# k-dominik/cluster_tools

Hardware: AMD Instinct MI355X
Metric: Gvoxel/s DT-watershed (node, 1/2/4/8 GPU) + % HBM roofline; VI vs ref (higher is better)
Workload: dtype f32

## Files before the change

### cluster_tools_amd/csrc/ctws_api.cpp

```cpp
#include <hip/hip_runtime.h>

#include <algorithm>
#include <chrono>
#include <type_traits>
#include <cmath>
#include <cstdint>
#include <cstdlib>
#include <cstdio>
#include <climits>
#include <cstring>
#include <memory>
#include <string>
#include <thread>
#include <utility>
#include <vector>

#include "../../include/ctws.h"
#include "ctws_kernels.h"
#include "host_pool.h"

using namespace ctws;

namespace {

// ... 64 lines not shown
        hipEvent_t ev_t0 = nullptr, ev_t1 = nullptr;
        std::vector<hipEvent_t> ev_blk;
    } hslot[2];
    hipStream_t s_in = nullptr, s_out = nullptr;
    DevBuf rl_lab, rl_bits, rl_cnt, rl_offs, rl_out, rl_keys, rl_vals, rl_red;
    DevBuf rl_sorted, rl_uniq, rl_counts, rl_tmp;
    int64_t rl_ntable = 0;
    DevBuf edt_fh;
    DevBuf xface;
    DevBuf ptile;
    DevBuf edt_scratch;
    DevBuf fs_vals, fs_sorted, fs_off, fs_tmp;
    DevBuf sf_ids, sf_bits, sf_desc, sf_stat, sf_seeds, sf_lab, sf_hm, sf_out;
    DevBuf rg_lab, rg_tab, rg_nodes, rg_pairs, rg_w, rg_keys, rg_skeys, rg_sw, rg_sum, rg_out, rg_tmp, rg_red;
    DevBuf ef_lab, ef_data, ef_nodes, ef_edges, ef_out, ef_ekeys, ef_keys, ef_skeys, ef_tmp, ef_red;
    DevBuf ov_lab, ov_rows;
    DevBuf mo_rows, mo_acc;
    DevBuf rf_data, rf_rows, rf_cnt, rf_off, rf_sums, rf_ctab;
    DevBuf ds_in, ds_out, ds_flag;
    std::vector<uint32_t> ds_flags;
    DevBuf rc_lab, rc_objs, rc_list, rc_keys, rc_cent, rc_found, rc_a, rc_b;
    DevBuf if_in, if_out, if_a, if_b, if_taps, if_mm;
    std::vector<double> if_taps_host;
    int64_t sf_n = 0;
    uint64_t sf_lo = 1, sf_hi = 0;
    bool sf_has_bits = false;
    DevBuf tc_P, tc_bits, tc_cnt, tc_offs, tc_woff, tc_red, tc_in, tc_mask, tc_out, tc_raw, tc_tmp, tc_taps;
    DevBuf ev_ka, ev_ca, ev_kb, ev_cb, ev_kp, ev_cp, ev_state, ev_out, ev_stage;
    int64_t ev_cap_a = 0, ev_cap_b = 0, ev_cap_p = 0;
    int stop_after = 0;
    int trace = 0;
    int no_descent = 0;
    int seed_tilecc = 0;
    int no_fallback = 0;
    int force_wide = 0;
    int wide_rerun = 0;
    int sf_sparse = 1;
    int fuse_hist = 1;
    int verify = 1;
    int prep_lds = 0;
    int plateau_fill = 1;
    int output_tile = 1;
    int gauss_w = 0;
    int gauss_yx = 1;
    int words_per_wave = 32;
    int d2h_wgs = 0;
    int pack_threads = 6;
    int unpack_threads = 9;
    std::unique_ptr<ctws_host::WorkerPool> pack_pool, unpack_pool;
    int h2d_mode = 0;
    int h2d_wgs = 64;
    int host_ramp = 1;
    int host_batch_blocks = 0;
    int64_t host_batch_voxels = (int64_t)256 << 20;
    int edt_wz = 0;
    int edt_bits = 1;
    int edt_w = 0;
    int fchunk2[3] = {1, 64, 1};
    int fchunk3[3] = {1, 8, 8};
    int fchunk3_masked[3] = {1, 8, 8};
    int fchunk3_env = 0;
    int fc_cur[3] = {1, 64, 1};
    int cur_max[3] = {0, 0, 0};
    int frontier_grid = 1024;
    int frontier_dir = 1;
    int frontier_reps = 32;
// ... 894 lines not shown
        if (edt_bits && maxX <= 256)
            launch_co(std::integral_constant<int, 4>(), std::true_type());
        else if (edt_bits && maxX <= 512)
            launch_co(std::integral_constant<int, 8>(), std::true_type());
        else if (edt_bits)
            launch_co(std::integral_constant<int, 16>(), std::true_type());
        else if (typed && all_exact && maxX == 256) {
            prep_kernel = 200 + 4;
            k_prep_edt_x_reg<4><<<gx, 256, 0, h->stream>>>(w.desc, w.stat, pp, fin_out, (uint32_t*)w.A);
        } else if (typed && all_exact && maxX == 512) {
            prep_kernel = 200 + 8;
            k_prep_edt_x_reg<8><<<gx, 256, 0, h->stream>>>(w.desc, w.stat, pp, fin_out, (uint32_t*)w.A);
        } else if (typed && all_exact && maxX == 1024) {
            prep_kernel = 200 + 16;
            k_prep_edt_x_reg<16><<<gx, 256, 0, h->stream>>>(w.desc, w.stat, pp, fin_out, (uint32_t*)w.A);
        } else if (typed && maxX <= 256)
            launch_co(std::integral_constant<int, 4>(), std::false_type());
        else if (typed && maxX <= 512)
            launch_co(std::integral_constant<int, 8>(), std::false_type());
        else if (typed && maxX <= 1024)
            launch_co(std::integral_constant<int, 16>(), std::false_type());
        else {
            lds_optin(k_prep_edt_x, 4 * (size_t)maxX * 4);
            k_prep_edt_x<<<gx, 256, 4 * (size_t)maxX * 4, h->stream>>>(w.desc, w.stat, pp, fin_out, (uint32_t*)w.A);
        }
        LAUNCHCHK();
        if (pl.from_seeds) k_fs_active<<<(nb + 255) / 256, 256, 0, h->stream>>>(w.desc, w.stat, nb);
        else k_set_active<<<(nb + 255) / 256, 256, 0, h->stream>>>(w.desc, w.stat, nb);
        LAUNCHCHK();
    }
    mark("prep_edt_x");
    set_timing(h, "prep_kernel", (float)prep_kernel);
    bool packed = true;
    uint32_t max_seeds = 0;
    std::vector<BlockStat> s2(nb);
    const dim3 gsb((unsigned)((maxZ + 255) / 256), nb);
    if (pl.from_seeds) {
        r = pl.sf_fill ? fs_seeds(h, desc, nb, TH, TW, TS, maxH, maxRows, vg, wg, uint64_t())
                       : fs_seeds(h, desc, nb, TH, TW, TS, maxH, maxRows, vg, wg, uint32_t());
        if (r != CTWS_OK) return r;
    } else {
    if (real_edt) {
        EdtRealParams er{{pl.pitchd[0], pl.pitchd[1], pl.pitchd[2]}, pl.dt_2d, real_double ? 1 : 0};
        const int nthr = 64 * 256;
        const int maxL = std::max(maxZ, std::max(maxY, maxX));
        const size_t esz = real_double ? 8 : 4;
        if ((r = grow(h, h->edt_scratch, (size_t)nthr * maxL * (2 * esz + 20))) != CTWS_OK) return r;
        char* scr = (char*)h->edt_scratch.p;
        auto run_real = [&](auto tag) {
            using T = decltype(tag);
            T* tmp = (T*)w.key;
            k_edt_real_init<T><<<vg, 256, 0, h->stream>>>(w.desc, w.stat, er, (const uint32_t*)w.A, tmp);
            for (int a = pl.dt_2d ? 1 : 0; a < 3; ++a)
                k_edt_real_line<T><<<nthr / 256, 256, 0, h->stream>>>(w.desc, w.stat, nb, er, a, tmp, scr, maxL);
            k_edt_real_final<T><<<vg, 256, 0, h->stream>>>(w.desc, w.stat, er, tmp, w.dt, w.smin, w.smax);
        };
        if (real_double) run_real(double());
        else run_real(float());
        LAUNCHCHK();
        if (!pl.dt_2d && pl.nd_ws == 2) {
            dim3 gs((unsigned)maxZ, nb);
            k_dt_slice_stats<<<gs, 256, 0, h->stream>>>(w.desc, w.stat, w.dt, w.smin, w.smax);
            LAUNCHCHK();
        }
    } else {
        auto fit = [](int W, int L) {
// ... 57 lines not shown
        std::fprintf(stderr, "[ctws] edt lower-envelope columns: y %u z %u\n", c[0], c[1]);
    }
    if (pl.pass2 && pl.nd_ws == 2) {
        k_p2_zero_dt<<<vg, 256, 0, h->stream>>>(w.desc, w.stat, w.dt);
        HIPCHK(hipMemsetD32Async((hipDeviceptr_t)w.smin, 0xFFFFFFFFu, (size_t)TS, h->stream));
        HIPCHK(hipMemsetAsync(w.smax, 0, sizeof(uint32_t) * TS, h->stream));
        dim3 gs((unsigned)maxZ, nb);
        k_dt_slice_stats<<<gs, 256, 0, h->stream>>>(w.desc, w.stat, w.dt, w.smin, w.smax);
        LAUNCHCHK();
    }
    mark("edt_yz");

    HmapParams hp{(float)cfg->alpha, (float)(1.0 - cfg->alpha), pl.nd_ws == 2 ? 1 : 0};
    const float* seedmap = w.dt;
    if (pl.seeds_smooth) {
        bool any = false;
        for (int a = (pl.nd_ws == 3 ? 0 : 1); a < 3; ++a) any |= pl.sig_seeds[a] > 0.0;
        if (any) {
            if ((r = run_gauss(h, pl, pl.sig_seeds, false, w.dt, w.sm, nb, maxZ, maxY, maxX, hp, 0)) != CTWS_OK)
                return r;
            seedmap = w.sm;
        }
    }
    mark("smooth_seeds");
    {
        const double sw[3] = {pl.weights_smooth ? pl.sig_weights[0] : 0.0, pl.weights_smooth ? pl.sig_weights[1] : 0.0,
                              pl.weights_smooth ? pl.sig_weights[2] : 0.0};
        if ((r = run_gauss(h, pl, sw, true, w.fin, w.hm, nb, maxZ, maxY, maxX, hp, 1)) != CTWS_OK) return r;
    }
    mark("hmap");

    {
        HIPCHK(hipMemsetAsync(h->ptile.p, 0, sizeof(uint32_t) * (size_t)std::max<int64_t>(TPT, 1), h->stream));
        k_localmax<<<wtg, 256, 0, h->stream>>>(w.desc, w.stat, seedmap, w.cls, w.smax, (uint32_t*)h->ptile.p);
        LAUNCHCHK();
        HIPCHK(hipMemsetAsync(w.fseed, 0, sizeof(uint64_t) * (size_t)TF, h->stream));
        CcArgs ca{seedmap, w.cls, w.P, nullptr, nullptr, 0, w.fseed, nullptr, (const uint32_t*)h->ptile.p};
        if (pl.nd_ws == 3) {
            using T = CcTileM<3, CC_SEED>;
            const dim3 tg(tiles8(cdiv(maxZ, T::TZ) * cdiv(maxY, T::TY) * cdiv(maxX, T::TX)), nb);
            k_tile_cc<3, CC_PLATEAU><<<tg, 256, 0, h->stream>>>(w.desc, w.stat, ca, w.P);
            k_tile_merge<3, CC_PLATEAU><<<dim3(std::min(tg.x, 2048u), tg.y), 256, 0, h->stream>>>(w.desc, w.stat, ca, w.P);
            k_plateau_flag<<<vg, 256, 0, h->stream>>>(w.desc, w.stat, w.cls, w.P);
            if (h->seed_tilecc) {
                k_tile_cc<3, CC_SEED><<<tg, 256, 0, h->stream>>>(w.desc, w.stat, ca, w.PF);
                k_tile_merge<3, CC_SEED><<<dim3(std::min(tg.x, 2048u), tg.y), 256, 0, h->stream>>>(w.desc, w.stat, ca, w.PF);
            } else {
                k_seed_members<3><<<wtg, 256, 0, h->stream>>>(w.desc, w.stat, w.cls, w.P, w.PF, w.fseed, nullptr);
            }
        } else {
            using T = CcTile<2>;
            const dim3 tg(tiles8(cdiv(maxZ, T::TZ) * cdiv(maxY, T::TY) * cdiv(maxX, T::TX)), nb);
            k_tile_cc<2, CC_PLATEAU><<<tg, 256, 0, h->stream>>>(w.desc, w.stat, ca, w.P);
            k_tile_merge<2, CC_PLATEAU><<<dim3(std::min(tg.x, 2048u), tg.y), 256, 0, h->stream>>>(w.desc, w.stat, ca, w.P);
            k_plateau_flag<<<vg, 256, 0, h->stream>>>(w.desc, w.stat, w.cls, w.P);
            if (h->seed_tilecc) {
                k_tile_cc<2, CC_SEED><<<tg, 256, 0, h->stream>>>(w.desc, w.stat, ca, w.PF);
                k_tile_merge<2, CC_SEED><<<dim3(std::min(tg.x, 2048u), tg.y), 256, 0, h->stream>>>(w.desc, w.stat, ca, w.PF);
            } else {
                k_seed_members<2><<<wtg, 256, 0, h->stream>>>(w.desc, w.stat, w.cls, w.P, w.PF, w.fseed,
                                                             (uint32_t*)w.A);
                k_seed_union2<<<dim3(64, nb), 256, 0, h->stream>>>(w.desc, w.stat, w.cls, w.P, (const uint32_t*)w.A,
                                                                   w.PF);
            }
        }
        LAUNCHCHK();
    }
    HIPCHK(hipMemsetAsync(w.W, 0, sizeof(uint64_t) * (size_t)TW, h->stream));
    k_flatten_seeds<<<dim3((unsigned)std::min<int64_t>((TF / nb + 255) / 256 + 1, 4096), nb), 256, 0, h->stream>>>(
        w.desc, w.stat, w.PF, w.fseed, w.W);
    k_bitmap_csum<<<wg, 256, 0, h->stream>>>(w.desc, w.stat, 0, w.W, w.csum);
    k_chunk_scan<<<nb, 256, 0, h->stream>>>(w.desc, w.stat, 0, w.csum, 0);
    k_word_prefix<<<wg, 256, 0, h->stream>>>(w.desc, w.stat, 0, w.W, w.csum, w.Wp);
    k_root_label<<<wg, 256, 0, h->stream>>>(w.desc, w.stat, 0, w.PF, w.W, w.Wp, pl.pass2 ? nullptr : (uint32_t*)w.Bf);
    if (pl.pass2) {
        k_slice_seed_base<<<gsb, 256, 0, h->stream>>>(w.desc, w.stat, w.W, w.Wp, w.soff);
        HIPCHK(hipMemsetAsync(w.hkey, 0xFF, sizeof(uint64_t) * (size_t)TH, h->stream));
        HIPCHK(hipMemsetAsync(w.hpos, 0xFF, sizeof(uint32_t) * (size_t)TH, h->stream));
        k_p2_insert<<<vg, 256, 0, h->stream>>>(w.desc, w.stat, w.hkey, w.hpos, w.PF, w.fseed, w.soff,
                                               (const uint32_t*)h->p2_hint_dev.p);
        HIPCHK(hipMemsetAsync(w.W, 0, sizeof(uint64_t) * (size_t)TW, h->stream));
        const dim3 hg((unsigned)std::min<int64_t>((maxH + 255) / 256, 4096), nb);
        k_p2_roots<<<hg, 256, 0, h->stream>>>(w.desc, w.stat, w.hkey, w.hpos, w.W);
        k_bitmap_csum<<<wg, 256, 0, h->stream>>>(w.desc, w.stat, 0, w.W, w.csum);
        k_chunk_scan<<<nb, 256, 0, h->stream>>>(w.desc, w.stat, 0, w.csum, 0);
        k_word_prefix<<<wg, 256, 0, h->stream>>>(w.desc, w.stat, 0, w.W, w.csum, w.Wp);
        k_root_label<<<wg, 256, 0, h->stream>>>(w.desc, w.stat, 0, nullptr, w.W, w.Wp, (uint32_t*)w.dt);
        LAUNCHCHK();
    }
    }
    {
        HIPCHK(hipMemcpyAsync(s2.data(), w.stat, sizeof(BlockStat) * nb, hipMemcpyDeviceToHost, h->stream));
        HIPCHK(hipStreamSynchronize(h->stream));
        for (auto& s : s2) {
// ... 391 lines not shown
        }
        if (any_plain) k_count_ids<<<dim3(64, nb), 256, 0, h->stream>>>(w.desc, w.stat, w.W);
        LAUNCHCHK();
        mark("output");
    }

    HIPCHK(hipMemcpyAsync(st.data(), w.stat, sizeof(BlockStat) * nb, hipMemcpyDeviceToHost, h->stream));
    std::vector<uint32_t> sbh, inmask, soffh;
    if (pl.pass2) {
        sbh.resize(TS);
        inmask.resize(TS);
        HIPCHK(hipMemcpyAsync(sbh.data(), w.sb, sizeof(uint32_t) * TS, hipMemcpyDeviceToHost, h->stream));
        HIPCHK(hipMemcpyAsync(inmask.data(), w.smin, sizeof(uint32_t) * TS, hipMemcpyDeviceToHost, h->stream));
        if (pl.nd_ws == 2) {
            soffh.resize(TS);
            HIPCHK(hipMemcpyAsync(soffh.data(), w.soff, sizeof(uint32_t) * TS, hipMemcpyDeviceToHost, h->stream));
        }
    }
    HIPCHK(hipStreamSynchronize(h->stream));
    for (size_t i = 1; i < ev; ++i) {
        float ms = 0.f;
        hipEventElapsedTime(&ms, h->events[i - 1], h->events[i]);
        add_timing(h, names[i], ms);
    }
    add_timing(h, "flood_rounds", (float)rounds1);
    add_timing(h, "frontier_iters", (float)fiters);
    add_timing(h, "regrow_iters", (float)fiters2);
    add_timing(h, "flood_fallback", (float)fallback);
    add_timing(h, "regrow_rounds", (float)rounds2);
    add_timing(h, "auto_seeded_blocks", (float)n_auto_blocks);
    add_timing(h, "sf_sparse_blocks", (float)n_sf_sparse);
    add_timing(h, "sf_redo_blocks", (float)n_sf_redo);
    add_timing(h, "hist_fused", counts_ready ? 1.f : 0.f);
    add_timing(h, "flood_kernel_ms", fk1);
    add_timing(h, "flood_packed", packed ? 1.f : 0.f);
    add_timing(h, "flood_tiles_solved", (float)h->flood_tiles);
    add_timing(h, "flood_local_iters", (float)h->flood_iters);
    add_timing(h, "flood_lines_swept", (float)h->flood_lines);
    add_timing(h, "size_filter_kernel_ms", fk2);
    std::vector<int> wide;
    if (packed)
        for (int i = 0; i < nb; ++i)
            if (st[i].active && st[i].dsat) wide.push_back(i);
    auto in_wide = [&](int i) { return std::find(wide.begin(), wide.end(), i) != wide.end(); };
    std::vector<int> redo;
    std::vector<std::vector<uint32_t>> redo_hint;
    if (pl.pass2 && pl.nd_ws == 2) {
        for (int i = 0; i < nb; ++i) {
            if (!st[i].active || in_wide(i)) continue;
            std::vector<uint32_t> so(soffh.begin() + desc[i].sbase, soffh.begin() + desc[i].sbase + desc[i].Z);
            const bool again = desc[i].p2hint < 0 ? (st[i].err & kErrCollision) != 0 : so != h->p2_hints[i];
            if (!again || (st[i].err & ~kErrCollision)) continue;
            if (h->p2_depth > desc[i].Z + 1) continue;
            redo.push_back(i);
            redo_hint.push_back(std::move(so));
        }
    }
    for (int i = 0; i < nb; ++i) {
        blocks[i].status = st[i].active ? CTWS_BLOCK_WRITTEN : (pl.pass2 ? CTWS_BLOCK_EMPTY_PASS2 : CTWS_BLOCK_EMPTY);
        blocks[i].max_label = st[i].active ? st[i].max_label : 0;
        if (pl.from_seeds) {
            uint64_t mx;
            std::memcpy(&mx, &st[i]._p[2], sizeof(mx));
            blocks[i].max_label = mx;
        }
        const uint32_t bare = (st[i].active ? st[i]._p[0] : 1u) && desc[i].id_offset != 0;
// ... 501 lines not shown
            for (int i = 0; i < nb; ++i)
                io[i] = {bb[i].input, bb[i].mask, bb[i].initial_seeds, bb[i].output};
            if ((r = run_batch(h, cfg, pl, bb.data(), io.data(), nb)) != CTWS_OK) return r;
        } else {
            if ((r = run_batch(h, cfg, pl, bb.data(), io.data(), nb)) != CTWS_OK) return r;
        }
        for (int i = 0; i < nb; ++i) {
            blocks[todo[k + i]].status = bb[i].status;
            blocks[todo[k + i]].n_ids = bb[i].n_ids;
            blocks[todo[k + i]].max_label = bb[i].max_label;
        }
        k = e;
    }
    return CTWS_OK;
}

}

extern "C" {

int ctws_abi_version(void) { return CTWS_ABI_VERSION; }

int ctws_open(int device, ctws_handle** out) {
    if (!out) return CTWS_EINVAL;
    *out = nullptr;
    int n = 0;
    if (hipGetDeviceCount(&n) != hipSuccess || n <= 0) return CTWS_EHIP;
    if (device < 0 || device >= n) return CTWS_EINVAL;
    ctws_handle* h = new ctws_handle();
    h->device = device;
    if (const char* t = std::getenv("CTWS_TRACE")) h->trace = std::atoi(t);
    if (const char* t = std::getenv("CTWS_NO_DESCENT")) h->no_descent = std::atoi(t);
    if (const char* t = std::getenv("CTWS_SEED_TILECC")) h->seed_tilecc = std::atoi(t);
    if (const char* t = std::getenv("CTWS_NO_FALLBACK")) h->no_fallback = std::atoi(t);
    if (const char* t = std::getenv("CTWS_FORCE_WIDE")) h->force_wide = std::atoi(t);
    if (const char* t = std::getenv("CTWS_SF_SPARSE")) h->sf_sparse = std::atoi(t);
    if (const char* t = std::getenv("CTWS_FUSE_HIST")) h->fuse_hist = std::atoi(t);
    if (const char* t = std::getenv("CTWS_VERIFY")) h->verify = std::atoi(t);
    if (const char* t = std::getenv("CTWS_PREP_LDS")) h->prep_lds = std::atoi(t);
    if (const char* t = std::getenv("CTWS_EDT_BITS")) h->edt_bits = std::atoi(t);
    if (const char* t = std::getenv("CTWS_FRONTIER_ITERS"))
        h->frontier_max_iters = std::max(0, std::min(kFrontierMaxItersCap, std::atoi(t)));
    if (const char* t = std::getenv("CTWS_GAUSS_YX")) h->gauss_yx = std::atoi(t);
    if (const char* t = std::getenv("CTWS_HOST_BATCH_VOXELS")) h->host_batch_voxels = std::max<int64_t>(1, std::atoll(t));
    if (const char* t = std::getenv("CTWS_HOST_RAMP")) h->host_ramp = std::atoi(t);
    if (const char* t = std::getenv("CTWS_PLATEAU_FILL")) h->plateau_fill = std::atoi(t);
    if (const char* t = std::getenv("CTWS_OUTPUT_TILE")) h->output_tile = std::atoi(t);
    if (const char* t = std::getenv("CTWS_H2D_MODE")) h->h2d_mode = std::atoi(t);
    if (const char* t = std::getenv("CTWS_H2D_WGS")) h->h2d_wgs = std::max(1, std::atoi(t));
    if (const char* t = std::getenv("CTWS_HOST_BATCH_BLOCKS")) h->host_batch_blocks = std::max(0, std::atoi(t));
    if (const char* t = std::getenv("CTWS_PACK_THREADS")) h->pack_threads = std::max(1, std::atoi(t));
    if (const char* t = std::getenv("CTWS_UNPACK_THREADS")) h->unpack_threads = std::max(1, std::atoi(t));
    if (const char* t = std::getenv("CTWS_D2H_WGS")) h->d2h_wgs = std::max(0, std::atoi(t));
    if (const char* t = std::getenv("CTWS_WORDS_PER_WAVE")) h->words_per_wave = std::max(1, std::atoi(t));
    if (const char* t = std::getenv("CTWS_GAUSS_W")) {
        const int v = std::atoi(t);
        h->gauss_w = (v == 8 || v == 16 || v == 32) ? v : 0;
    }
    if (const char* t = std::getenv("CTWS_EDT_W")) {
        const int v = std::atoi(t);
        h->edt_w = (v == 8 || v == 16 || v == 32 || v == 64) ? v : 0;
    }
    if (const char* t = std::getenv("CTWS_EDT_WZ")) {
        const int v = std::atoi(t);
        h->edt_wz = (v == 8 || v == 16 || v == 32 || v == 64) ? v : 0;
    }
// ... 2222 lines not shown
```

### cluster_tools_amd/csrc/ctws_kernels.h

```cpp
#pragma once

#include "ctws_dev.h"

namespace ctws {

struct PrepParams {
    float threshold;
    int invert;
    int agg;
    int px2;
};
struct EdtColParams {
    int axis;
    int p2;
    int final_pass;
    int per_slice;
    uint32_t max_dist;
    int px2;
};
struct EdtRealParams {
    double pitch[3];
    int per_slice;
    int real;
};
// ... 29 lines not shown
__global__ void k_edt_col_bits(const BlockDesc*, BlockStat*, EdtColParams, const EdtRec*, uint32_t*, float*, uint32_t*,
                               uint32_t*, unsigned long long*, uint32_t*);
__global__ void k_edt_col_fh(const BlockDesc*, BlockStat*, EdtColParams, const uint32_t*, const EdtRec*, uint32_t*,
                             float*, uint32_t*, uint32_t*, const unsigned long long*, const uint32_t*);
template <class T>
__global__ void k_edt_real_init(const BlockDesc*, const BlockStat*, EdtRealParams, const uint32_t*, T*);
template <class T>
__global__ void k_edt_real_line(const BlockDesc*, const BlockStat*, int, EdtRealParams, int, T*, char*, int);
template <class T>
__global__ void k_edt_real_final(const BlockDesc*, BlockStat*, EdtRealParams, const T*, float*, uint32_t*, uint32_t*);
__global__ void k_dt_slice_stats(const BlockDesc*, const BlockStat*, const float*, uint32_t*, uint32_t*);
__global__ void k_set_active(const BlockDesc*, BlockStat*, int);

__global__ void k_hmap(const BlockDesc*, const BlockStat*, HmapParams, const float*, const float*, const uint32_t*,
                       const uint32_t*, float*);
template <int W>
__global__ void k_gauss_col(const BlockDesc*, const BlockStat*, GaussParams, HmapParams, const double*, const float*,
                            const float*, const uint32_t*, const uint32_t*, float*);
__global__ void k_gauss_row(const BlockDesc*, const BlockStat*, GaussParams, HmapParams, const double*, const float*,
                            const float*, const uint32_t*, const uint32_t*, float*);
constexpr int kTapSlot = 4096;
constexpr int kGaussMaxR = 12;
template <int W, int R>
__global__ void k_gauss_col_r(const BlockDesc*, const BlockStat*, GaussParams, HmapParams, const double*, const float*,
                              const float*, const uint32_t*, const uint32_t*, float*);
template <int R>
__global__ void k_gauss_row_r(const BlockDesc*, const BlockStat*, GaussParams, HmapParams, const double*, const float*,
                              const float*, const uint32_t*, const uint32_t*, float*);
constexpr int kGaussYxTY = 32;
template <int R>
__global__ void k_gauss_yx(const BlockDesc*, const BlockStat*, int, HmapParams, const double*, const double*,
                           const float*, const float*, const uint32_t*, const uint32_t*, float*);

__global__ void k_localmax(const BlockDesc*, BlockStat*, const float*, uint8_t*, const uint32_t*, uint32_t*);
__global__ void k_plateau_flag(const BlockDesc*, const BlockStat*, uint8_t*, uint32_t*);
__global__ void k_flatten_tile_roots(const BlockDesc*, const BlockStat*, uint32_t*, const uint64_t*, uint64_t*);
__global__ void k_flatten_seeds(const BlockDesc*, const BlockStat*, uint32_t*, const uint64_t*, uint64_t*);
template <int ND>
__global__ void k_seed_members(const BlockDesc*, BlockStat*, const uint8_t*, const uint32_t*, uint32_t*, uint64_t*,
                               uint32_t*);
__global__ void k_seed_union2(const BlockDesc*, const BlockStat*, const uint8_t*, const uint32_t*, const uint32_t*,
                              uint32_t*);

__global__ void k_plat_mark(const BlockDesc*, const BlockStat*, const float*, const uint32_t*, uint64_t*, uint64_t*);
template <int ND>
__global__ void k_plat_entry(const BlockDesc*, const BlockStat*, const float*, uint64_t*, const uint64_t*,
                             const uint32_t*);
__global__ void k_plat_scan_x(const BlockDesc*, const BlockStat*, uint64_t*, const uint64_t*, const uint32_t*);
template <int AX>
__global__ void k_plat_scan_col(const BlockDesc*, const BlockStat*, uint64_t*, const uint64_t*, const uint32_t*);
__global__ void k_plat_restore(const BlockDesc*, const BlockStat*, uint64_t*, const uint64_t*, uint64_t*);
__global__ void k_bitmap_csum(const BlockDesc*, const BlockStat*, int, const uint64_t*, uint32_t*);
__global__ void k_chunk_scan(const BlockDesc*, BlockStat*, int, uint32_t*, int);
__global__ void k_word_prefix(const BlockDesc*, const BlockStat*, int, const uint64_t*, const uint32_t*, uint32_t*);
__global__ void k_root_label(const BlockDesc*, const BlockStat*, int, uint32_t*, const uint64_t*, const uint32_t*,
                             uint32_t*);
__global__ void k_seed_label(const BlockDesc*, const BlockStat*, const uint32_t*, const uint64_t*, const float*,
                             uint32_t*, uint64_t*, uint8_t*, int);
__global__ void k_output(const BlockDesc*, BlockStat*, const uint32_t*, const uint64_t*, int, const uint32_t*,
                         const uint32_t*, const uint32_t*, unsigned long long*, int);
__global__ void k_count_ids(const BlockDesc*, BlockStat*, const uint64_t*);

enum CcMode { CC_PLATEAU = 0, CC_SEED = 1, CC_CROP = 2 };
struct CcArgs {
    const float* v;
    const uint8_t* cls;
    const uint32_t* Pp;
    const uint32_t* lab;
// ... 335 lines not shown
```

### cluster_tools_amd/csrc/k_cc.hip

```cpp
#include "ctws_kernels.h"

namespace ctws {

#define BLOCK_LOOP(i, B)                                                                      \
    for (int64_t i = (int64_t)blockIdx.x * blockDim.x + threadIdx.x; i < (B).N;              \
         i += (int64_t)gridDim.x * blockDim.x)

#define ROW_TILES(nz, ny, nx, ...)                                                           \
    {                                                                                         \
        const int64_t nrows_ = (int64_t)(nz) * (ny);                                          \
        for (int64_t r0_ = (int64_t)blockIdx.x * kRows; r0_ < nrows_; r0_ += (int64_t)gridDim.x * kRows) \
            for (int x = threadIdx.x; x < (nx); x += blockDim.x) {                           \
                _Pragma("unroll") for (int rr_ = 0; rr_ < kRows; ++rr_) {                      \
                    const int64_t row_ = r0_ + rr_;                                           \
                    if (row_ >= nrows_) break;                                                \
                    const int z = (int)(row_ / (ny));                                         \
                    const int y = (int)(row_ - (int64_t)z * (ny));                            \
                    const int64_t i = row_ * (nx) + x;                                        \
                    (void)z;                                                                  \
                    (void)y;                                                                  \
                    __VA_ARGS__                                                               \
                }                                                                             \
            }                                                                                 \
    }

template <int ND>
__device__ __forceinline__ void localmax_words(const BlockDesc& B, const BlockStat& st, const uint32_t* __restrict__ smax,
                                               const float* __restrict__ p, uint8_t* __restrict__ cl, uint32_t& nplat,
                                               uint32_t* __restrict__ ptile) {
    const uint32_t ord0 = 0x80000000u;
    constexpr int U = 8, R = U + 2;
    const int Y = B.Y, X = B.X, Z = B.Z;
    const int64_t YX = (int64_t)Y * X;
    const int wpr = (X + 63) >> 6;
    const int ngy = (Y + U - 1) / U;
    const int64_t nunits = (int64_t)Z * wpr * ngy;
    const int lane = threadIdx.x & 63;
    const int64_t nwaves = (int64_t)gridDim.x * (blockDim.x >> 6);
    const int64_t per = (nunits + nwaves - 1) / nwaves;
    const int64_t wid = (int64_t)xcd_swizzle((int)blockIdx.x, (int)gridDim.x) * (blockDim.x >> 6) + (threadIdx.x >> 6);
    const int64_t ubeg = wid * per, uend = min(nunits, ubeg + per);
    const float NEG = -__builtin_huge_valf();
    const gptr_t<float> gp = gbl(p);
    for (int64_t un = ubeg; un < uend; ++un) {
        const uint32_t un32 = (uint32_t)un;
        const int gy = (int)(un32 % (uint32_t)ngy);
        const uint32_t strip = un32 / (uint32_t)ngy;
        const int xw = (int)(strip % (uint32_t)wpr), z = (int)(strip / (uint32_t)wpr);
        const int y0 = gy * U;
        bool ueq = false;
        const int x = xw * 64 + lane;
        const int xc = min(x, X - 1);
        const int xe = lane == 0 ? max(xc - 1, 0) : min(xc + 1, X - 1);
        const int64_t zb = (int64_t)z * YX;
        float rc[R], re[R];
#pragma unroll
        for (int k = 0; k < R; ++k) {
            const int yy = min(max(y0 - 1 + k, 0), Y - 1);
            rc[k] = gp[zb + (int64_t)yy * X + xc];
            re[k] = gp[zb + (int64_t)yy * X + xe];
        }
        float zm[U], zp[U];
// ... 34 lines not shown
            float w[8];
            if (ND == 3) {
                w[0] = z > 0 ? zm[u] : NEG;
                w[1] = z + 1 < Z ? zp[u] : NEG;
                w[2] = yl ? rc[k - 1] : NEG;
                w[3] = yh ? rc[k + 1] : NEG;
                w[4] = xl ? lft[k] : NEG;
                w[5] = xh ? rgt[k] : NEG;
                w[6] = w[7] = NEG;
            } else {
                w[0] = yl && xl ? lft[k - 1] : NEG;
                w[1] = yl ? rc[k - 1] : NEG;
                w[2] = yl && xh ? rgt[k - 1] : NEG;
                w[3] = xl ? lft[k] : NEG;
                w[4] = xh ? rgt[k] : NEG;
                w[5] = yh && xl ? lft[k + 1] : NEG;
                w[6] = yh ? rc[k + 1] : NEG;
                w[7] = yh && xh ? rgt[k + 1] : NEG;
            }
            bool gt = false, eq = false;
#pragma unroll
            for (int q = 0; q < 8; ++q) {
                gt |= w[q] > cc;
                eq |= w[q] == cc;
            }
            if (cc == 0.0f && pos) {
                gt = true;
                eq = false;
            }
            const bool valid = y < Y && x < X;
            if (valid) cl[zb + (int64_t)y * X + x] = (uint8_t)((gt ? 1 : 0) | (eq ? 2 : 0));
            nplat += valid && eq;
            ueq |= valid && eq;
        }
        const uint64_t em = __ballot(ueq);
        if (em && lane < (ND == 3 ? 2 : 1)) {
            using PT = CcTileM<ND, CC_PLATEAU>;
            const int ntx = (X + PT::TX - 1) / PT::TX, nty = (Y + PT::TY - 1) / PT::TY;
            const uint64_t half = ND == 3 ? ((em >> (32 * lane)) & 0xFFFFFFFFull) : em;
            const int txi = ND == 3 ? 2 * xw + lane : xw;
            if (half && txi < ntx) {
                uint32_t* f = ptile + B.ptbase + ((int64_t)(z / PT::TZ) * nty + y0 / PT::TY) * ntx + txi;
                if (!*f) *f = 1u;
            }
        }
    }
}

__global__ void __launch_bounds__(256) k_localmax(const BlockDesc* __restrict__ D, BlockStat* S,
                                                  const float* __restrict__ v, uint8_t* __restrict__ cls,
                                                  const uint32_t* __restrict__ smax, uint32_t* __restrict__ ptile) {
    const BlockDesc& B = D[blockIdx.y];
    if (!S[blockIdx.y].active) return;
    uint32_t nplat = 0;
    if (B.nd_ws == 3) localmax_words<3>(B, S[blockIdx.y], smax, v + B.base, cls + B.base, nplat, ptile);
    else localmax_words<2>(B, S[blockIdx.y], smax, v + B.base, cls + B.base, nplat, ptile);
    nplat = wg_reduce_u32(nplat, OpAdd());
    if (threadIdx.x == 0 && nplat) atomicAdd(&S[blockIdx.y].plateau, nplat);
}

template <int ND>
__global__ void __launch_bounds__(256) k_seed_members(const BlockDesc* __restrict__ D, BlockStat* S,
                                                      const uint8_t* __restrict__ cls, const uint32_t* __restrict__ Pp,
                                                      uint32_t* __restrict__ PFg, uint64_t* __restrict__ fseed,
                                                      uint32_t* __restrict__ plist) {
    const BlockDesc& B = D[blockIdx.y];
    BlockStat& st = S[blockIdx.y];
    if (!st.active) return;
    const bool plat = st.plateau != 0;
    const uint8_t* cl = cls + B.base;
    const uint32_t* PP = Pp + B.base;
    uint32_t* PF = PFg + B.base;
    const int wpr = (B.X + 63) >> 6;
    const int64_t nwords = (int64_t)B.Z * B.Y * wpr;
    const int lane = threadIdx.x & 63;
    const int64_t nwaves = (int64_t)gridDim.x * (blockDim.x >> 6);
    const int64_t per = (nwords + nwaves - 1) / nwaves;
    const int64_t wid = (int64_t)xcd_swizzle((int)blockIdx.x, (int)gridDim.x) * (blockDim.x >> 6) + (threadIdx.x >> 6);
    const int64_t wbeg = wid * per, wend = min(nwords, wbeg + per);
    int row_n = (int)((uint32_t)wbeg / (uint32_t)wpr), xw_n = (int)(wbeg - (int64_t)row_n * wpr);
    constexpr int U = 8;
    for (int64_t w0 = wbeg; w0 < wend; w0 += U) {
        int64_t gi[U];
        bool valid[U];
        uint8_t c[U];
#pragma unroll
        for (int u = 0; u < U; ++u) {
            const int64_t row = row_n;
            const int x = xw_n * 64 + lane;
// ... 76 lines not shown
    const uint32_t n = st._u;
    for (uint32_t e = blockIdx.x * blockDim.x + threadIdx.x; e < n; e += gridDim.x * blockDim.x) {
        const uint32_t i = plist[B.base + e];
        const uint32_t x = i % (uint32_t)B.X, y = (i / (uint32_t)B.X) % (uint32_t)B.Y;
        if (x > 0 && plat_max(i - 1)) unite(i, i - 1);
        if (y > 0 && plat_max(i - (uint32_t)B.X)) unite(i, i - (uint32_t)B.X);
    }
}

__global__ void __launch_bounds__(256) k_plateau_flag(const BlockDesc* __restrict__ D, const BlockStat* S,
                                                      uint8_t* __restrict__ cls, uint32_t* __restrict__ Pg) {
    const BlockDesc& B = D[blockIdx.y];
    if (!S[blockIdx.y].active || !S[blockIdx.y].plateau) return;
    uint8_t* cl = cls + B.base;
    uint32_t* P = Pg + B.base;
    const int64_t a0 = B.base >> 4, a1 = (B.base + B.N + 15) >> 4;
    const uint4* c16 = reinterpret_cast<const uint4*>(cls);
    for (int64_t a = a0 + (int64_t)blockIdx.x * blockDim.x + threadIdx.x; a < a1; a += (int64_t)gridDim.x * blockDim.x) {
        const uint4 q = c16[a];
        const uint32_t wv[4] = {q.x, q.y, q.z, q.w};
#pragma unroll
        for (int k = 0; k < 4; ++k) {
            uint32_t m = wv[k] & (wv[k] >> 1) & 0x01010101u;
            while (m) {
                const int b = __builtin_ctz(m) >> 3;
                m &= m - 1u;
                const int64_t i = a * 16 + k * 4 + b - B.base;
                if (i < 0 || i >= B.N) continue;
                const uint32_t r = uf_find_compress(P, (uint32_t)i);
                cl[r] |= 4;
            }
        }
    }
}

__global__ void __launch_bounds__(256) k_bitmap_csum(const BlockDesc* __restrict__ D, const BlockStat* S, int inner,
                                                     const uint64_t* __restrict__ Wg, uint32_t* __restrict__ csum) {
    const BlockDesc& B = D[blockIdx.y];
    if (!S[blockIdx.y].active || (inner && !B.crop)) return;
    const int64_t n = inner ? B.NI : B.N;
    const int64_t nw = n / 64 + 1;
    if ((int64_t)blockIdx.x * 256 >= nw) return;
    const int64_t w = (int64_t)blockIdx.x * 256 + threadIdx.x;
    uint32_t c = w < nw ? (uint32_t)__popcll(Wg[B.wbase + w]) : 0u;
    for (int s = 32; s > 0; s >>= 1) c += (uint32_t)__shfl_xor((int)c, s);
    __shared__ uint32_t red[4];
    if ((threadIdx.x & 63) == 0) red[threadIdx.x >> 6] = c;
    __syncthreads();
    if (threadIdx.x == 0) csum[B.cbase + blockIdx.x] = red[0] + red[1] + red[2] + red[3];
}

__global__ void __launch_bounds__(256) k_chunk_scan(const BlockDesc* __restrict__ D, BlockStat* S, int inner,
                                                    uint32_t* __restrict__ csum, int which_counter) {
    const BlockDesc& B = D[blockIdx.x];
    if (!S[blockIdx.x].active || (inner && !B.crop)) return;
    const int64_t n = inner ? B.NI : B.N;
    const int64_t nw = n / 64 + 1;
    const int64_t nc = (nw + 255) / 256;
    __shared__ uint32_t tmp[256];
    uint32_t carry = 0;
    for (int64_t c0 = 0; c0 < nc; c0 += 256) {
        const int64_t c = c0 + threadIdx.x;
        uint32_t v = c < nc ? csum[B.cbase + c] : 0u;
        tmp[threadIdx.x] = v;
        __syncthreads();
        for (int s = 1; s < 256; s <<= 1) {
// ... 310 lines not shown
```

Measured before the change: 17.52.

## Emit seed and plateau bitmaps from localmax and process only plateau words

k_localmax now writes per-word ballots of strict local maxima into fseed and of plateau voxels into a new feq bitmap, and writes PF for strict maxima directly. Plateau flagging and seed membership then walk only the nonzero feq words instead of scanning every voxel, and the fseed memset is skipped. The aim is to remove dense full-volume passes over cls in the seed stage. The cost is extra ballot work and global writes inside localmax, plus a new path whose correctness depends on fseed and PF staying consistent. The old dense path stays behind CTWS_SEED_DENSE.

```diff
diff --git a/cluster_tools_amd/csrc/ctws_api.cpp b/cluster_tools_amd/csrc/ctws_api.cpp
--- a/cluster_tools_amd/csrc/ctws_api.cpp
+++ b/cluster_tools_amd/csrc/ctws_api.cpp
@@ -120,6 +120,7 @@
     int trace = 0;
     int no_descent = 0;
     int seed_tilecc = 0;
+    int seed_dense = 0;
     int no_fallback = 0;
     int force_wide = 0;
     int wide_rerun = 0;
@@ -1080,6 +1081,7 @@
     mark("prep_edt_x");
     set_timing(h, "prep_kernel", (float)prep_kernel);
     bool packed = true;
+    const bool seed_dense = !pl.from_seeds && (h->seed_dense || h->seed_tilecc);
     uint32_t max_seeds = 0;
     std::vector<BlockStat> s2(nb);
     const dim3 gsb((unsigned)((maxZ + 255) / 256), nb);
@@ -1203,34 +1205,48 @@
 
     {
         HIPCHK(hipMemsetAsync(h->ptile.p, 0, sizeof(uint32_t) * (size_t)std::max<int64_t>(TPT, 1), h->stream));
-        k_localmax<<<wtg, 256, 0, h->stream>>>(w.desc, w.stat, seedmap, w.cls, w.smax, (uint32_t*)h->ptile.p);
+        const bool dense = seed_dense;
+        uint64_t* const feq = w.fopen;
+        if (dense) k_localmax<<<wtg, 256, 0, h->stream>>>(w.desc, w.stat, seedmap, w.cls, w.smax, (uint32_t*)h->ptile.p,
+                                                         nullptr, nullptr, nullptr);
+        else k_localmax<<<wtg, 256, 0, h->stream>>>(w.desc, w.stat, seedmap, w.cls, w.smax, (uint32_t*)h->ptile.p,
+                                                    w.fseed, feq, w.PF);
         LAUNCHCHK();
-        HIPCHK(hipMemsetAsync(w.fseed, 0, sizeof(uint64_t) * (size_t)TF, h->stream));
+        if (dense) HIPCHK(hipMemsetAsync(w.fseed, 0, sizeof(uint64_t) * (size_t)TF, h->stream));
         CcArgs ca{seedmap, w.cls, w.P, nullptr, nullptr, 0, w.fseed, nullptr, (const uint32_t*)h->ptile.p};
+        const dim3 eg((unsigned)std::min<int64_t>((maxRows * ((maxX + 63) / 64) + 255) / 256, 2048), nb);
         if (pl.nd_ws == 3) {
             using T = CcTileM<3, CC_SEED>;
             const dim3 tg(tiles8(cdiv(maxZ, T::TZ) * cdiv(maxY, T::TY) * cdiv(maxX, T::TX)), nb);
             k_tile_cc<3, CC_PLATEAU><<<tg, 256, 0, h->stream>>>(w.desc, w.stat, ca, w.P);
             k_tile_merge<3, CC_PLATEAU><<<dim3(std::min(tg.x, 2048u), tg.y), 256, 0, h->stream>>>(w.desc, w.stat, ca, w.P);
-            k_plateau_flag<<<vg, 256, 0, h->stream>>>(w.desc, w.stat, w.cls, w.P);
+            if (dense) k_plateau_flag<<<vg, 256, 0, h->stream>>>(w.desc, w.stat, w.cls, w.P);
+            else k_plateau_flag_eq<<<eg, 256, 0, h->stream>>>(w.desc, w.stat, w.cls, w.P, feq);
             if (h->seed_tilecc) {
                 k_tile_cc<3, CC_SEED><<<tg, 256, 0, h->stream>>>(w.desc, w.stat, ca, w.PF);
                 k_tile_merge<3, CC_SEED><<<dim3(std::min(tg.x, 2048u), tg.y), 256, 0, h->stream>>>(w.desc, w.stat, ca, w.PF);
+            } else if (dense) {
+                k_seed_members<3><<<wtg, 256, 0, h->stream>>>(w.desc, w.stat, w.cls, w.P, w.PF, w.fseed, nullptr);
             } else {
-                k_seed_members<3><<<wtg, 256, 0, h->stream>>>(w.desc, w.stat, w.cls, w.P, w.PF, w.fseed, nullptr);
+                k_seed_members_eq<3><<<eg, 256, 0, h->stream>>>(w.desc, w.stat, w.cls, w.P, w.PF, w.fseed, feq, nullptr);
             }
         } else {
             using T = CcTile<2>;
             const dim3 tg(tiles8(cdiv(maxZ, T::TZ) * cdiv(maxY, T::TY) * cdiv(maxX, T::TX)), nb);
             k_tile_cc<2, CC_PLATEAU><<<tg, 256, 0, h->stream>>>(w.desc, w.stat, ca, w.P);
             k_tile_merge<2, CC_PLATEAU><<<dim3(std::min(tg.x, 2048u), tg.y), 256, 0, h->stream>>>(w.desc, w.stat, ca, w.P);
-            k_plateau_flag<<<vg, 256, 0, h->stream>>>(w.desc, w.stat, w.cls, w.P);
+            if (dense) k_plateau_flag<<<vg, 256, 0, h->stream>>>(w.desc, w.stat, w.cls, w.P);
+            else k_plateau_flag_eq<<<eg, 256, 0, h->stream>>>(w.desc, w.stat, w.cls, w.P, feq);
             if (h->seed_tilecc) {
                 k_tile_cc<2, CC_SEED><<<tg, 256, 0, h->stream>>>(w.desc, w.stat, ca, w.PF);
                 k_tile_merge<2, CC_SEED><<<dim3(std::min(tg.x, 2048u), tg.y), 256, 0, h->stream>>>(w.desc, w.stat, ca, w.PF);
             } else {
-                k_seed_members<2><<<wtg, 256, 0, h->stream>>>(w.desc, w.stat, w.cls, w.P, w.PF, w.fseed,
-                                                             (uint32_t*)w.A);
+                if (dense)
+                    k_seed_members<2><<<wtg, 256, 0, h->stream>>>(w.desc, w.stat, w.cls, w.P, w.PF, w.fseed,
+                                                                 (uint32_t*)w.A);
+                else
+                    k_seed_members_eq<2><<<eg, 256, 0, h->stream>>>(w.desc, w.stat, w.cls, w.P, w.PF, w.fseed, feq,
+                                                                   (uint32_t*)w.A);
                 k_seed_union2<<<dim3(64, nb), 256, 0, h->stream>>>(w.desc, w.stat, w.cls, w.P, (const uint32_t*)w.A,
                                                                    w.PF);
             }
@@ -1688,6 +1704,7 @@
     add_timing(h, "sf_sparse_blocks", (float)n_sf_sparse);
     add_timing(h, "sf_redo_blocks", (float)n_sf_redo);
     add_timing(h, "hist_fused", counts_ready ? 1.f : 0.f);
+    add_timing(h, "seed_dense", seed_dense ? 1.f : 0.f);
     add_timing(h, "flood_kernel_ms", fk1);
     add_timing(h, "flood_packed", packed ? 1.f : 0.f);
     add_timing(h, "flood_tiles_solved", (float)h->flood_tiles);
@@ -2255,6 +2272,7 @@
     if (const char* t = std::getenv("CTWS_TRACE")) h->trace = std::atoi(t);
     if (const char* t = std::getenv("CTWS_NO_DESCENT")) h->no_descent = std::atoi(t);
     if (const char* t = std::getenv("CTWS_SEED_TILECC")) h->seed_tilecc = std::atoi(t);
+    if (const char* t = std::getenv("CTWS_SEED_DENSE")) h->seed_dense = std::atoi(t);
     if (const char* t = std::getenv("CTWS_NO_FALLBACK")) h->no_fallback = std::atoi(t);
     if (const char* t = std::getenv("CTWS_FORCE_WIDE")) h->force_wide = std::atoi(t);
     if (const char* t = std::getenv("CTWS_SF_SPARSE")) h->sf_sparse = std::atoi(t);
diff --git a/cluster_tools_amd/csrc/ctws_kernels.h b/cluster_tools_amd/csrc/ctws_kernels.h
--- a/cluster_tools_amd/csrc/ctws_kernels.h
+++ b/cluster_tools_amd/csrc/ctws_kernels.h
@@ -85,8 +85,13 @@
 __global__ void k_gauss_yx(const BlockDesc*, const BlockStat*, int, HmapParams, const double*, const double*,
                            const float*, const float*, const uint32_t*, const uint32_t*, float*);
 
-__global__ void k_localmax(const BlockDesc*, BlockStat*, const float*, uint8_t*, const uint32_t*, uint32_t*);
+__global__ void k_localmax(const BlockDesc*, BlockStat*, const float*, uint8_t*, const uint32_t*, uint32_t*, uint64_t*,
+                           uint64_t*, uint32_t*);
 __global__ void k_plateau_flag(const BlockDesc*, const BlockStat*, uint8_t*, uint32_t*);
+__global__ void k_plateau_flag_eq(const BlockDesc*, const BlockStat*, uint8_t*, uint32_t*, const uint64_t*);
+template <int ND>
+__global__ void k_seed_members_eq(const BlockDesc*, BlockStat*, const uint8_t*, const uint32_t*, uint32_t*, uint64_t*,
+                                  const uint64_t*, uint32_t*);
 __global__ void k_flatten_tile_roots(const BlockDesc*, const BlockStat*, uint32_t*, const uint64_t*, uint64_t*);
 __global__ void k_flatten_seeds(const BlockDesc*, const BlockStat*, uint32_t*, const uint64_t*, uint64_t*);
 template <int ND>
diff --git a/cluster_tools_amd/csrc/k_cc.hip b/cluster_tools_amd/csrc/k_cc.hip
--- a/cluster_tools_amd/csrc/k_cc.hip
+++ b/cluster_tools_amd/csrc/k_cc.hip
@@ -27,7 +27,8 @@
 template <int ND>
 __device__ __forceinline__ void localmax_words(const BlockDesc& B, const BlockStat& st, const uint32_t* __restrict__ smax,
                                                const float* __restrict__ p, uint8_t* __restrict__ cl, uint32_t& nplat,
-                                               uint32_t* __restrict__ ptile) {
+                                               uint32_t* __restrict__ ptile, uint64_t* __restrict__ fseed,
+                                               uint64_t* __restrict__ feq, uint32_t* __restrict__ PF) {
     const uint32_t ord0 = 0x80000000u;
     constexpr int U = 8, R = U + 2;
     const int Y = B.Y, X = B.X, Z = B.Z;
@@ -128,6 +129,16 @@
             if (valid) cl[zb + (int64_t)y * X + x] = (uint8_t)((gt ? 1 : 0) | (eq ? 2 : 0));
             nplat += valid && eq;
             ueq |= valid && eq;
+            if (fseed) {
+                const bool smx = valid && !gt && !eq;
+                const uint64_t ms = __ballot(smx), me = __ballot(valid && eq);
+                if (y < Y && lane == 0) {
+                    const int64_t fw = B.fbase + ((int64_t)z * Y + y) * wpr + xw;
+                    fseed[fw] = ms;
+                    feq[fw] = me;
+                }
+                if (smx) PF[zb + (int64_t)y * X + x] = (uint32_t)(zb + (int64_t)y * X + x);
+            }
         }
         const uint64_t em = __ballot(ueq);
         if (em && lane < (ND == 3 ? 2 : 1)) {
@@ -145,12 +156,15 @@
 
 __global__ void __launch_bounds__(256) k_localmax(const BlockDesc* __restrict__ D, BlockStat* S,
                                                   const float* __restrict__ v, uint8_t* __restrict__ cls,
-                                                  const uint32_t* __restrict__ smax, uint32_t* __restrict__ ptile) {
+                                                  const uint32_t* __restrict__ smax, uint32_t* __restrict__ ptile,
+                                                  uint64_t* __restrict__ fseed, uint64_t* __restrict__ feq,
+                                                  uint32_t* __restrict__ PFg) {
     const BlockDesc& B = D[blockIdx.y];
     if (!S[blockIdx.y].active) return;
     uint32_t nplat = 0;
-    if (B.nd_ws == 3) localmax_words<3>(B, S[blockIdx.y], smax, v + B.base, cls + B.base, nplat, ptile);
-    else localmax_words<2>(B, S[blockIdx.y], smax, v + B.base, cls + B.base, nplat, ptile);
+    uint32_t* PF = PFg ? PFg + B.base : nullptr;
+    if (B.nd_ws == 3) localmax_words<3>(B, S[blockIdx.y], smax, v + B.base, cls + B.base, nplat, ptile, fseed, feq, PF);
+    else localmax_words<2>(B, S[blockIdx.y], smax, v + B.base, cls + B.base, nplat, ptile, fseed, feq, PF);
     nplat = wg_reduce_u32(nplat, OpAdd());
     if (threadIdx.x == 0 && nplat) atomicAdd(&S[blockIdx.y].plateau, nplat);
 }
@@ -293,6 +307,85 @@
             }
         }
     }
+}
+
+#define EQ_WORDS(B, feq, cl, ...)                                                                \
+    {                                                                                             \
+        const int wpr = ((B).X + 63) >> 6;                                                        \
+        const int64_t nwords_ = (int64_t)(B).Z * (B).Y * wpr;                                     \
+        const int lane = threadIdx.x & 63;                                                        \
+        const int64_t nwaves_ = (int64_t)gridDim.x * (blockDim.x >> 6);                           \
+        const int64_t wave_ = (int64_t)blockIdx.x * (blockDim.x >> 6) + (threadIdx.x >> 6);       \
+        for (int64_t w0_ = wave_ * 64; w0_ < nwords_; w0_ += nwaves_ * 64) {                      \
+            const uint64_t e_ = w0_ + lane < nwords_ ? gbl(feq)[(B).fbase + w0_ + lane] : 0ull;   \
+            uint64_t nz_ = __ballot(e_ != 0ull);                                                  \
+            while (nz_) {                                                                         \
+                const int64_t w = w0_ + __builtin_ctzll(nz_);                                     \
+                nz_ &= nz_ - 1ull;                                                                \
+                const uint32_t row_ = (uint32_t)w / (uint32_t)wpr;                                \
+                const int x = ((int)((uint32_t)w - row_ * (uint32_t)wpr) << 6) + lane;            \
+                const bool valid = x < (B).X;                                                     \
+                const int64_t gi = valid ? (int64_t)row_ * (B).X + x : 0;                         \
+                const uint8_t c = valid ? (cl)[gi] : (uint8_t)1;                                  \
+                __VA_ARGS__                                                                       \
+            }                                                                                     \
+        }                                                                                         \
+    }
+
+template <int ND>
+__global__ void __launch_bounds__(256) k_seed_members_eq(const BlockDesc* __restrict__ D, BlockStat* S,
+                                                         const uint8_t* __restrict__ cls, const uint32_t* __restrict__ Pp,
+                                                         uint32_t* __restrict__ PFg, uint64_t* __restrict__ fseed,
+                                                         const uint64_t* __restrict__ feq, uint32_t* __restrict__ plist) {
+    const BlockDesc& B = D[blockIdx.y];
+    BlockStat& st = S[blockIdx.y];
+    if (!st.active || !st.plateau) return;
+    const uint8_t* cl = cls + B.base;
+    const uint32_t* PP = Pp + B.base;
+    uint32_t* PF = PFg + B.base;
+    EQ_WORDS(B, feq, cl, {
+        bool mx = !(c & 1);
+        uint32_t par = (uint32_t)gi;
+        bool listed = false;
+        if (mx && (c & 2)) {
+            const uint32_t r = uf_find(PP, par);
+            if (cl[r] & 4) mx = false;
+            else if (ND == 3) par = r;
+            else listed = true;
+        }
+        const uint64_t m = __ballot(mx);
+        if (lane == 0) fseed[B.fbase + w] = m;
+        if (mx) PF[gi] = par;
+        if (ND == 2) {
+            const uint64_t lm = __ballot(listed);
+            if (lm) {
+                uint32_t base = 0;
+                if (lane == 0) base = atomicAdd(&st._u, (uint32_t)__popcll(lm));
+                base = (uint32_t)__shfl((int)base, 0);
+                if (listed) plist[B.base + base + __popcll(lm & ((1ull << lane) - 1ull))] = par;
+            }
+        }
+    })
+}
+template __global__ void k_seed_members_eq<2>(const BlockDesc*, BlockStat*, const uint8_t*, const uint32_t*, uint32_t*,
+                                              uint64_t*, const uint64_t*, uint32_t*);
+template __global__ void k_seed_members_eq<3>(const BlockDesc*, BlockStat*, const uint8_t*, const uint32_t*, uint32_t*,
+                                              uint64_t*, const uint64_t*, uint32_t*);
+
+__global__ void __launch_bounds__(256) k_plateau_flag_eq(const BlockDesc* __restrict__ D, const BlockStat* S,
+                                                         uint8_t* __restrict__ cls, uint32_t* __restrict__ Pg,
+                                                         const uint64_t* __restrict__ feq) {
+    const BlockDesc& B = D[blockIdx.y];
+    if (!S[blockIdx.y].active || !S[blockIdx.y].plateau) return;
+    uint8_t* cl = cls + B.base;
+    uint32_t* P = Pg + B.base;
+    EQ_WORDS(B, feq, cl, {
+        (void)w;
+        if ((c & 3) == 3) {
+            const uint32_t r = uf_find_compress(P, (uint32_t)gi);
+            cl[r] |= 4;
+        }
+    })
 }
 
 __global__ void __launch_bounds__(256) k_bitmap_csum(const BlockDesc* __restrict__ D, const BlockStat* S, int inner,
```

Measured after the change: 17.80 (median of 6 runs). +1.6%, better.
